# mandt-lab/PSLD

Measured on AMD Instinct MI355X. Metric: train images/sec, CIFAR-10 PSLD (6ch 32x32) NCSN++ HSM step, higher is better.
Workload: dtype f32

## Files before the change

### psld_amd/csrc/conv_wino.hip

```cpp
#include <cstdlib>
#include <cstring>
#include <type_traits>

#include "common.h"
#include "psld_hip.h"
#include "tile_shared.h"
#include "limb.h"

namespace {

constexpr int WT = 32;
constexpr int VPLANE = WT * ROWB;
constexpr int VBYTES = 16 * 3 * VPLANE;
constexpr int WINO_THREADS = 512;

struct WinoArgs {
    const float* x1;
    const float* x2;
    int C1, C2;
    int B, H, W;
    const u32x4* ufrag;
    int N, M;
    int chunks;
    float* C;
    int ldc;
    int nseg, rps;
    int cw;
    PsldEpilogue e;
    const float* zero;
    int nmajor;
    int tiles_m;
    int stagger;
    const float *gsc1, *gsh1, *gsc2, *gsh2;
    int gn_act;
    unsigned long long* dbg;
    int lg_tiles_x, lg_tps;
    int ksplit;
    long long slab_stride;
    int lg_ksplit, lg_xblocks;
    int lg_rpi;
    int mul_seg, mul_w2;
    int rb_img;
    float opscale;
};

constexpr int wino_mul16(int d) { return 65536 / d + 1; }
__host__ __device__ constexpr int wino_div16(int x, int mul) { return (x * mul) >> 16; }
constexpr int WINO_GEOS[6][2] = {{4, 8}, {8, 8}, {16, 8}, {4, 16}, {8, 16}, {4, 32}};
constexpr bool wino_div16_exact() {
    for (const auto& g : WINO_GEOS) {
        const int W2 = g[1] + 2, seg_px = (g[0] + 2) * W2;
        for (int x = 0; x < 256; ++x)
            if (wino_div16(x, wino_mul16(seg_px)) != x / seg_px || wino_div16(x, wino_mul16(W2)) != x / W2) return false;
    }
    return true;
}
static_assert(wino_div16_exact(), "halo decomposition: multiply-shift must equal the division for every pixel below 256");
constexpr bool wino_geo_listed(int rps, int cw) {
    for (const auto& g : WINO_GEOS)
        if (g[0] == rps && g[1] == cw) return true;
    return false;
}
constexpr int wino_lg2(int v) {
    int l = 0;
    while ((1 << l) < v) ++l;
    return (1 << l) == v ? l : -1;
}

__device__ __forceinline__ int raw_off(int hp, int q) {
    return (hp >> 1) * 256 + (((((hp & 1) ^ ((hp >> 1) & 1)) << 3) + q) << 4);
}

template <int NL = 3>
__device__ __forceinline__ void wino_pack_item(const float* __restrict__ w, u32x4* __restrict__ out, long long it, int k_in,
                                               long long sn, long long sk, int flip) {
    const int chunks = k_in / 32;
    long long t = it;
    const int lane = (int)(t & 63); t >>= 6;
    const int chunk = (int)(t % chunks); t /= chunks;
    const int nblk = (int)t;
    const int n = nblk * 16 + (lane & 15);
    const int k0 = chunk * 32 + (lane >> 4) * 8;
    float U[8][16];
#pragma unroll
    for (int j = 0; j < 8; ++j) {
        const float* p = w + n * sn + (k0 + j) * sk;
        float g[3][3];
#pragma unroll
        for (int a = 0; a < 3; ++a)
#pragma unroll
            for (int b = 0; b < 3; ++b) g[a][b] = flip ? p[8 - (a * 3 + b)] : p[a * 3 + b];
        float t4[4][3];
#pragma unroll
        for (int b = 0; b < 3; ++b) {
            t4[0][b] = g[0][b];
            t4[1][b] = 0.5f * ((g[0][b] + g[2][b]) + g[1][b]);
            t4[2][b] = 0.5f * ((g[0][b] + g[2][b]) - g[1][b]);
            t4[3][b] = g[2][b];
        }
#pragma unroll
        for (int a = 0; a < 4; ++a) {
            U[j][a * 4 + 0] = t4[a][0];
            U[j][a * 4 + 1] = 0.5f * ((t4[a][0] + t4[a][2]) + t4[a][1]);
            U[j][a * 4 + 2] = 0.5f * ((t4[a][0] + t4[a][2]) - t4[a][1]);
            U[j][a * 4 + 3] = t4[a][2];
        }
    }
    u32x4* o = out + ((long long)nblk * chunks + chunk) * (16 * NL * 64) + lane;
#pragma unroll
    for (int p = 0; p < 16; ++p) {
        unsigned hi[4], mid[4], lo[4];
#pragma unroll
        for (int j = 0; j < 4; ++j) {
            if constexpr (NL == 3) split3(U[2 * j][p], U[2 * j + 1][p], hi[j], mid[j], lo[j]);
            else if constexpr (NL == 2) split2(U[2 * j][p], U[2 * j + 1][p], hi[j], mid[j]);
            else hi[j] = cvt_pk_f16(U[2 * j][p], U[2 * j + 1][p]);
        }
        o[(p * NL + 0) * 64] = u32x4{hi[0], hi[1], hi[2], hi[3]};
        if constexpr (NL >= 2) o[(p * NL + 1) * 64] = u32x4{mid[0], mid[1], mid[2], mid[3]};
        if constexpr (NL == 3) o[(p * 3 + 2) * 64] = u32x4{lo[0], lo[1], lo[2], lo[3]};
    }
}

template <int NL = 3>
__global__ void wino_pack_kernel(const float* __restrict__ w, u32x4* __restrict__ out, int n_out, int k_in,
                                 long long sn, long long sk, int flip) {
    const long long items = (long long)(n_out / 16) * (k_in / 32) * 64;
    for (long long it = (long long)blockIdx.x * blockDim.x + threadIdx.x; it < items; it += (long long)gridDim.x * blockDim.x)
        wino_pack_item<NL>(w, out, it, k_in, sn, sk, flip);
}

template <int NL = 3>
__global__ void wino_pack_batch_kernel(const long long* __restrict__ tab, int ntab, long long total) {
    for (long long idx = (long long)blockIdx.x * blockDim.x + threadIdx.x; idx < total;
         idx += (long long)gridDim.x * blockDim.x) {
        int lo = 0, hi = ntab - 1;
        while (lo < hi) {
            const int mid = (lo + hi + 1) >> 1;
            if (tab[8 * mid + 7] <= idx) lo = mid; else hi = mid - 1;
        }
        const long long* d = tab + 8 * lo;
        wino_pack_item<NL>(reinterpret_cast<const float*>(d[0]), reinterpret_cast<u32x4*>(d[1]), idx - d[7], (int)d[3], d[5], d[6],
                       (int)d[4]);
    }
}

template <int ABL = 0, bool GNF = false, bool ERAW = false, int LA = 2, bool TAIL = false, int NL = 3, bool SH = false>
__global__ void __launch_bounds__(WINO_THREADS) wino_conv8s_kernel(const WinoArgs a) {
    extern __shared__ __attribute__((aligned(16))) unsigned char smem[];
    constexpr int NI = 4;
    constexpr int RAWB = NI * 64 * 128;
    unsigned char* Vs = smem;
    unsigned char* Rs = smem + VBYTES / 3 * NL;

    const int tid = threadIdx.x;
    const int lane = tid & 63, wave = __builtin_amdgcn_readfirstlane(tid >> 6);
    const int tiles_n = TAIL ? (a.N + 127) >> 7 : a.N >> 7;
    const int nsp = a.ksplit > 1 ? a.ksplit : 1;
    const int tiles_m = a.tiles_m;
    const int per_range = tiles_m * tiles_n;
    const int vb = xcd_remap(blockIdx.x, gridDim.x);
    const int split = nsp > 1 ? vb / per_range : 0;
    const int bid = vb - split * per_range;
    const int kch = a.chunks >> a.lg_ksplit, ch0 = split * kch;
    float* const Cw = a.C + split * a.slab_stride;
    const int tile_n = a.nmajor ? bid / tiles_m : bid % tiles_n;
    const int tile_m = a.nmajor ? bid - tile_n * tiles_m : bid / tiles_n;
    const int n0 = tile_n * 128;
    const bool live = !TAIL || n0 + wave * 16 < a.N;

    const int HW = a.H * a.W;
    const int W2 = a.cw + 2;
    const int lg_tx = a.lg_tiles_x, lg_tps = a.lg_tps;
    const int rpi = HW >= 128 ? HW >> 7 : 1;
    const int tm_img = a.lg_rpi >= 0 ? tile_m >> a.lg_rpi : tile_m / rpi;
    const int reg = tile_m - tm_img * rpi;
    const int img0 = HW >= 128 ? tm_img : tile_m * a.nseg;
    const int oy0 = (reg >> a.lg_xblocks) * a.rps, ox0 = (reg & ((1 << a.lg_xblocks) - 1)) * a.cw;
    const float* zp = a.zero;

    const int c4 = tid & 7;
    int hoff[NI], rdst[NI];
    {
        const int seg_px = (a.rps + 2) * W2;
#pragma unroll
        for (int i = 0; i < NI; ++i) {
            const int px = (tid + WINO_THREADS * i) >> 3;
            const int seg = wino_div16(px, a.mul_seg);
            const int rem = px - seg * seg_px;
            const int hr = wino_div16(rem, a.mul_w2), hx = rem - hr * W2;
            const int img = img0 + seg, iy = oy0 + hr - 1, ix = ox0 + hx - 1;
            const bool ok = seg < a.nseg && img < a.B && iy >= 0 && iy < a.H && ix >= 0 && ix < a.W;
            hoff[i] = ok ? (img * a.H + iy) * a.W + ix : -1;
            rdst[i] = raw_off(px, c4);
        }
    }
    f32x4 hv[NI];
    auto load_raw = [&](int c) {
        const int c0 = c * 32;
        const bool second = c0 >= a.C1;
        const float* src = second ? a.x2 : a.x1;
        const int cs = second ? a.C2 : a.C1;
        const int cc = (second ? c0 - a.C1 : c0) + c4 * 4;
#pragma unroll
        for (int i = 0; i < NI; ++i) hv[i] = ld4(hoff[i] >= 0 ? src + ((long long)hoff[i] * cs + cc) : zp);
    };
    auto store_raw = [&](int buf, int c) {
        if constexpr (GNF) {
            const int c0 = c * 32;
            const bool second = c0 >= a.C1;
            const int cs = second ? a.C2 : a.C1;
            const long long go = (long long)img0 * cs + (second ? c0 - a.C1 : c0) + c4 * 4;
            const f32x4 sc = ld4((second ? a.gsc2 : a.gsc1) + go), sh = ld4((second ? a.gsh2 : a.gsh1) + go);
#pragma unroll
            for (int i = 0; i < NI; ++i) {
                f32x4 o;
#pragma unroll
                for (int e = 0; e < 4; ++e) {
                    const float z = hv[i][e] * sc[e] + sh[e];
                    const float v = a.gn_act ? silu_f(z) : z;
                    o[e] = hoff[i] >= 0 ? v : 0.f;
                }
                *reinterpret_cast<f32x4*>(Rs + buf * RAWB + rdst[i]) = o;
            }
        } else {
#pragma unroll
            for (int i = 0; i < NI; ++i) *reinterpret_cast<f32x4*>(Rs + buf * RAWB + rdst[i]) = hv[i];
        }
    };

    const int vr = wave >> 2;
    const int t_tile = (tid & 255) >> 3, t_q = tid & 7;
    int t_src;
    {
        const int seg = t_tile >> lg_tps, rem = t_tile & ((1 << lg_tps) - 1);
        const int ty = rem >> lg_tx, tx = rem & ((1 << lg_tx) - 1);
        t_src = (seg * (a.rps + 2) + 2 * ty) * W2 + 2 * tx;
    }
    const int t_dst = t_tile * ROWB + (((t_q >> 1) ^ lds_swz(t_tile)) << 4) + (t_q & 1) * 8;
    int t_ro[3][4];
#pragma unroll
    for (int k = 0; k < 3; ++k)
#pragma unroll
        for (int c = 0; c < 4; ++c) {
            t_ro[k][c] = raw_off(t_src + (vr + k) * W2 + c, t_q);
            asm volatile("" : "+v"(t_ro[k][c]));
        }
    auto transform = [&](auto TH, auto VR, int rbuf) {
        constexpr int th = decltype(TH)::value, v_r = decltype(VR)::value;
        constexpr int ra_ = th == 0 ? (v_r == 0 ? 0 : 1) : (v_r == 0 ? 2 : 1);
        constexpr int rb_ = th == 0 ? 2 : (v_r == 0 ? 1 : 3);
        constexpr bool plus = th == 0 && v_r == 1;
        constexpr int vrow = 2 * th + v_r;
        const unsigned char* Rb = Rs + rbuf * RAWB;
        f32x4 ea[4], eb[4];
#pragma unroll
        for (int c = 0; c < 4; ++c) {
            ea[c] = *reinterpret_cast<const f32x4*>(Rb + t_ro[ra_ - v_r][c]);
            eb[c] = *reinterpret_cast<const f32x4*>(Rb + t_ro[rb_ - v_r][c]);
        }
        f32x4 r[4];
#pragma unroll
        for (int c = 0; c < 4; ++c) r[c] = plus ? ea[c] + eb[c] : ea[c] - eb[c];
#pragma unroll
        for (int j = 0; j < 4; ++j) {
            const f32x4 v = j == 0 ? r[0] - r[2] : j == 1 ? r[1] + r[2] : j == 2 ? r[2] - r[1] : r[1] - r[3];
            unsigned h0, m0_, l0, h1, m1, l1;
            if constexpr (NL == 3) {
                split3(v[0], v[1], h0, m0_, l0);
                split3(v[2], v[3], h1, m1, l1);
            } else if constexpr (NL == 2) {
                split2(v[0], v[1], h0, m0_);
                split2(v[2], v[3], h1, m1);
            } else if constexpr (SH) {
                h0 = cvt_pk_f16(v[0] * a.opscale, v[1] * a.opscale);
                h1 = cvt_pk_f16(v[2] * a.opscale, v[3] * a.opscale);
            } else {
                h0 = cvt_pk_f16(v[0], v[1]);
                h1 = cvt_pk_f16(v[2], v[3]);
            }
            unsigned char* q = Vs + (vrow * 4 + j) * NL * VPLANE + t_dst;
            *reinterpret_cast<u32x2*>(q) = u32x2{h0, h1};
            if constexpr (NL >= 2) *reinterpret_cast<u32x2*>(q + VPLANE) = u32x2{m0_, m1};
            if constexpr (NL == 3) *reinterpret_cast<u32x2*>(q + 2 * VPLANE) = u32x2{l0, l1};
        }
    };

    const int r16 = lane & 15, kq = lane >> 4;
    int aoff[2];
#pragma unroll
    for (int tb = 0; tb < 2; ++tb) {
        const int row = tb * 16 + r16;
        aoff[tb] = row * ROWB + ((kq ^ lds_swz(row)) << 4);
    }
    const u32x4* ub = a.ufrag + ((long long)(tile_n * 8 + ((ABL & 128) ? (wave & 3) : wave)) * a.chunks + ch0) * (16 * NL * 64);
    u32x4 bq[4][NL];
    auto load_b = [&](int sigma, u32x4 (&dst)[NL]) {
        const u32x4* p = ub + (long long)sigma * (NL * 64);
#pragma unroll
        for (int l = 0; l < NL; ++l) dst[l] = p[l * 64 + lane];
    };
    f32x4v acc[16][2];
#pragma unroll
    for (int p = 0; p < 16; ++p)
#pragma unroll
        for (int tb = 0; tb < 2; ++tb) acc[p][tb] = f32x4v{0.f, 0.f, 0.f, 0.f};
    u32x4 fa[NL == 1 ? 2 : NL][2];
    auto read_a = [&](int p, int l) {
#pragma unroll
        for (int tb = 0; tb < 2; ++tb) fa[l][tb] = *reinterpret_cast<const u32x4*>(Vs + (p * NL + l) * VPLANE + aoff[tb]);
    };
    auto mm = [&](int p, int la, int lb) {
#pragma unroll
        for (int tb = 0; tb < 2; ++tb) {
            if constexpr (NL == 1)
                acc[p][tb] = __builtin_amdgcn_mfma_f32_16x16x32_f16(
                    __builtin_bit_cast(f16x8, bq[p & 3][lb]), __builtin_bit_cast(f16x8, fa[la][tb]), acc[p][tb], 0, 0, 0);
            else
                acc[p][tb] = __builtin_amdgcn_mfma_f32_16x16x32_bf16(
                    __builtin_bit_cast(bf16x8, bq[p & 3][lb]), __builtin_bit_cast(bf16x8, fa[la][tb]), acc[p][tb], 0, 0, 0);
        }
    };
    auto mfma_half = [&](auto HH, auto LAST, int c) {
        constexpr int h = decltype(HH)::value;
        constexpr bool last = decltype(LAST)::value;
        if constexpr ((ABL & 256) != 0) __builtin_amdgcn_s_setprio(2);
        if constexpr (NL == 1) {
            auto read_a1 = [&](int p) {
#pragma unroll
                for (int tb = 0; tb < 2; ++tb) fa[p & 1][tb] = *reinterpret_cast<const u32x4*>(Vs + p * VPLANE + aoff[tb]);
            };
            read_a1(8 * h);
#pragma unroll
            for (int i = 0; i < 8; ++i) {
                const int p = 8 * h + i;
                if (!(last && p + LA >= 16)) load_b(c * 16 + p + LA, bq[(p + LA) & 3]);
                if (i < 7) read_a1(p + 1);
                __builtin_amdgcn_sched_barrier(0);
                mm(p, p & 1, 0);
                __builtin_amdgcn_sched_barrier(0);
            }
            return;
        }
        if constexpr (NL == 3) read_a(8 * h, 2);
        if constexpr (NL >= 2) read_a(8 * h, 1);
        read_a(8 * h, 0);
#pragma unroll
        for (int i = 0; i < 8; ++i) {
            const int p = 8 * h + i;
            if (!(ABL & 2) && !(last && p + LA >= 16)) load_b(c * 16 + p + LA, bq[(p + LA) & 3]);
            __builtin_amdgcn_sched_barrier(0);
            if constexpr (NL == 3) {
                mm(p, 2, 0);
                __builtin_amdgcn_sched_barrier(0);
                if (i < 7) read_a(p + 1, 2);
                __builtin_amdgcn_sched_barrier(0);
                mm(p, 1, 1);
            }
            if constexpr (NL >= 2) {
                mm(p, 1, 0);
                __builtin_amdgcn_sched_barrier(0);
                if (i < 7) read_a(p + 1, 1);
                __builtin_amdgcn_sched_barrier(0);
            }
            if constexpr (NL == 3) mm(p, 0, 2);
            if constexpr (NL >= 2) mm(p, 0, 1);
            mm(p, 0, 0);
            __builtin_amdgcn_sched_barrier(0);
            if (i < 7) read_a(p + 1, 0);
        }
        if constexpr ((ABL & 256) != 0) __builtin_amdgcn_s_setprio(0);
    };
    using I0 = std::integral_constant<int, 0>;
    using I1 = std::integral_constant<int, 1>;
    if constexpr ((ABL & 4) == 0 && (ABL & 256) == 0) { if (vr != 0) __builtin_amdgcn_s_setprio(1); }

    load_raw(ch0);
    if (live) {
        load_b(0, bq[0]);
        load_b(1, bq[1]);
        if (LA > 2) load_b(2, bq[2]);
    }
    store_raw(0, ch0);
    if constexpr (ERAW) load_raw(ch0 + min(1, kch - 1));
    __syncthreads();
    if (vr == 0) transform(I0{}, I0{}, 0); else transform(I0{}, I1{}, 0);
    __syncthreads();

    auto stamp = [&](int c, int idx) {
        if constexpr ((ABL & 64) != 0) {
            if (c == 3 && a.dbg) {
                __builtin_amdgcn_sched_barrier(0);
                const unsigned long long t = __builtin_amdgcn_s_memtime();
                if (lane == 0) a.dbg[((long long)blockIdx.x * 8 + wave) * 8 + idx] = t;
                __builtin_amdgcn_sched_barrier(0);
            }
        }
    };
    using No = std::false_type;
    using Yes = std::true_type;

    for (int c = 0; c < kch - 1; ++c) {
        stamp(c, 0);
        if constexpr (!ERAW) load_raw(ch0 + c + 1);
        if (vr == 0 && !(ABL & 1)) transform(I1{}, I0{}, c & 1);
        __builtin_amdgcn_sched_barrier(0);
        if (vr == 0) stamp(c, 1);
        if (live) mfma_half(I0{}, No{}, c);
        __builtin_amdgcn_sched_barrier(0);
        if (vr != 0) stamp(c, 1);
        if (vr != 0 && !(ABL & 1)) transform(I1{}, I1{}, c & 1);
        stamp(c, 2);
        store_raw((c + 1) & 1, ch0 + c + 1);
        stamp(c, 3);
        __syncthreads();
        stamp(c, 4);
        if (vr == 0 && !(ABL & 1)) transform(I0{}, I0{}, (c + 1) & 1);
        __builtin_amdgcn_sched_barrier(0);
        if (vr == 0) stamp(c, 5);
        if (live) mfma_half(I1{}, No{}, c);
        __builtin_amdgcn_sched_barrier(0);
        if (vr != 0) stamp(c, 5);
        if constexpr (ERAW) load_raw(ch0 + min(c + 2, kch - 1));
        if (vr != 0 && !(ABL & 1)) transform(I0{}, I1{}, (c + 1) & 1);
        stamp(c, 6);
        __syncthreads();
        stamp(c, 7);
    }
    {
        int c = kch - 1;
        asm volatile("" : "+s"(c));
        stamp(c, 0);
        if (vr == 0 && !(ABL & 1)) transform(I1{}, I0{}, c & 1);
        __builtin_amdgcn_sched_barrier(0);
        if (vr == 0) stamp(c, 1);
        if (live) mfma_half(I0{}, No{}, c);
        __builtin_amdgcn_sched_barrier(0);
        if (vr != 0) stamp(c, 1);
        if (vr != 0 && !(ABL & 1)) transform(I1{}, I1{}, c & 1);
        stamp(c, 2);
        stamp(c, 3);
        __syncthreads();
        stamp(c, 4);
        __builtin_amdgcn_sched_barrier(0);
        stamp(c, 5);
        if (live) mfma_half(I1{}, Yes{}, c);
// ... 483 lines not shown
```

### psld_amd/csrc/pointwise.hip

```cpp
#include "common.h"
#include "psld_hip.h"

namespace {

inline int grid_for(long long n, int per_thread = 1) {
    long long b = (n + 256LL * per_thread - 1) / (256LL * per_thread);
    if (b > 256LL * 16) b = 256LL * 16;
    if (b < 1) b = 1;
    return (int)b;
}

#define GRID_STRIDE(i, n) \
    for (long long i = (long long)blockIdx.x * blockDim.x + threadIdx.x; i < (n); i += (long long)gridDim.x * blockDim.x)

__global__ void transpose_kernel(const float* __restrict__ x, float* __restrict__ y, int rows, int cols) {
    __shared__ float tile[32][33];
    const long long img = blockIdx.z;
    const float* xp = x + img * rows * cols;
    float* yp = y + img * rows * cols;
    const int c0 = blockIdx.x * 32, r0 = blockIdx.y * 32;
    const int tx = threadIdx.x & 31, ty = threadIdx.x >> 5;
    for (int j = ty; j < 32; j += 8) {
        const int r = r0 + j, c = c0 + tx;
        if (r < rows && c < cols) tile[j][tx] = xp[(long long)r * cols + c];
// ... 207 lines not shown
        const float* p = job.src + col;
        const long long step = 16ll * job.ld;
        int r = lane;
        for (; r + 7 * 16 < job.rows; r += 8 * 16) {
            float v[8];
            const float* q = p + (long long)r * job.ld;
#pragma unroll
            for (int u = 0; u < 8; ++u) v[u] = q[u * step];
#pragma unroll
            for (int u = 0; u < 8; ++u) acc += (double)v[u];
        }
        for (; r < job.rows; r += 16) acc += (double)p[(long long)r * job.ld];
    }
    sh[lane * 64 + (tid & 63)] = acc;
    __syncthreads();
    if (lane == 0 && col < job.c) {
        double t = 0.0;
#pragma unroll
        for (int l = 0; l < 16; ++l) t += sh[l * 64 + tid];
        const float v = (float)(t * (double)job.alpha);
        job.dst1[col] = v;
        if (job.dst2) job.dst2[col] = v;
    }
}

__global__ void im2col3x3_small_kernel(const float* __restrict__ x, int ih, int iw, int c, int oh, int ow, int stride,
                                       int pad, int flip, float* __restrict__ out, int ld_out, long long total) {
    GRID_STRIDE(i, total) {
        const int j = (int)(i % ld_out);
        const long long m = i / ld_out;
        float v = 0.f;
        if (j < 9 * c) {
            const int ch = j / 9;
            int t = j - ch * 9;
            if (flip) t = 8 - t;
            const int ky = t / 3, kx = t - ky * 3;
            const int ox = (int)(m % ow);
            const long long r = m / ow;
            const int oy = (int)(r % oh);
            const long long n = r / oh;
            const int iy = oy * stride + ky - pad, ix = ox * stride + kx - pad;
            if (iy >= 0 && iy < ih && ix >= 0 && ix < iw) v = x[((n * ih + iy) * iw + ix) * c + ch];
        }
        out[i] = v;
    }
}

__global__ void im2col3x3_kernel(const float* __restrict__ x, int ih, int iw, int c4, int oh, int ow, int stride, int pad,
                                 float* __restrict__ cols, long long total4) {
    GRID_STRIDE(i, total4) {
        const int q = (int)(i % c4);
        long long r = i / c4;
        const int t = (int)(r % 9);
        const long long m = r / 9;
        const int ky = t / 3, kx = t - ky * 3;
        const int ox = (int)(m % ow);
        const long long rr = m / ow;
        const int oy = (int)(rr % oh);
        const long long n = rr / oh;
        const int iy = oy * stride + ky - pad, ix = ox * stride + kx - pad;
        f32x4 v = {0.f, 0.f, 0.f, 0.f};
        if (iy >= 0 && iy < ih && ix >= 0 && ix < iw)
            v = reinterpret_cast<const f32x4*>(x)[((n * ih + iy) * iw + ix) * c4 + q];
        reinterpret_cast<f32x4*>(cols)[i] = v;
    }
}
__global__ void col2im3x3_kernel(const float* __restrict__ dcols, int ih, int iw, int c4, int oh, int ow, int stride,
                                 int pad, float* __restrict__ dx, long long total4) {
    GRID_STRIDE(i, total4) {
        const int q = (int)(i % c4);
        long long r = i / c4;
        const int ix = (int)(r % iw);
        r /= iw;
        const int iy = (int)(r % ih);
        const long long n = r / ih;
        f32x4 acc = {0.f, 0.f, 0.f, 0.f};
#pragma unroll
        for (int ky = 0; ky < 3; ++ky) {
            const int ty = iy + pad - ky;
            if (ty < 0 || ty % stride) continue;
            const int oy = ty / stride;
            if (oy >= oh) continue;
#pragma unroll
            for (int kx = 0; kx < 3; ++kx) {
                const int tx = ix + pad - kx;
                if (tx < 0 || tx % stride) continue;
                const int ox = tx / stride;
                if (ox >= ow) continue;
                const long long m = (n * oh + oy) * ow + ox;
                acc += reinterpret_cast<const f32x4*>(dcols)[(m * 9 + ky * 3 + kx) * c4 + q];
            }
        }
        reinterpret_cast<f32x4*>(dx)[i] = acc;
    }
}

template <int COUT>
__global__ void __launch_bounds__(256) conv3x3_fewout_kernel(const float* __restrict__ x, const float* __restrict__ w_ohwi,
                                                            const float* __restrict__ bias, float* __restrict__ y,
                                                            int batch, int h, int w, int c) {
    extern __shared__ __attribute__((aligned(16))) float wl[];
    for (int i = threadIdx.x; i < 9 * COUT * c; i += blockDim.x) {
        const int ch = i % c, r = i / c;
        const int o = r % COUT, t = r / COUT;
        wl[i] = w_ohwi[((long long)o * 9 + t) * c + ch];
    }
    __syncthreads();
    const int lane = threadIdx.x & 63, wave = threadIdx.x >> 6;
    const int c4 = c >> 2;
    const bool live = lane < c4;
    const int wq = (w + 3) >> 2;
    const long long groups = (long long)batch * h * wq;
    for (long long gidx = (long long)blockIdx.x * 4 + wave; gidx < groups; gidx += (long long)gridDim.x * 4) {
        const int gx = (int)(gidx % wq);
        const long long r = gidx / wq;
        const int oy = (int)(r % h);
        const long long n = r / h;
        const int ox0 = gx * 4;
        f32x4 win[3][6];
#pragma unroll
        for (int dy = 0; dy < 3; ++dy)
#pragma unroll
            for (int dx = 0; dx < 6; ++dx) {
                const int iy = oy + dy - 1, ix = ox0 + dx - 1;
                const bool ok = live && iy >= 0 && iy < h && ix >= 0 && ix < w;
                win[dy][dx] = ok ? reinterpret_cast<const f32x4*>(x)[((n * h + iy) * w + ix) * c4 + lane]
                                 : f32x4{0.f, 0.f, 0.f, 0.f};
            }
        float acc[4][COUT];
#pragma unroll
        for (int p = 0; p < 4; ++p)
#pragma unroll
            for (int o = 0; o < COUT; ++o) acc[p][o] = 0.f;
        if (live) {
#pragma unroll
            for (int t = 0; t < 9; ++t) {
                const int ky = t / 3, kx = t - ky * 3;
#pragma unroll
                for (int o = 0; o < COUT; ++o) {
                    const f32x4 wv = *reinterpret_cast<const f32x4*>(wl + ((t * COUT + o) * c) + lane * 4);
#pragma unroll
                    for (int p = 0; p < 4; ++p) {
                        const f32x4 xv = win[ky][p + kx];
                        float a = acc[p][o];
                        a = fmaf(xv[0], wv[0], a);
                        a = fmaf(xv[1], wv[1], a);
                        a = fmaf(xv[2], wv[2], a);
                        a = fmaf(xv[3], wv[3], a);
                        acc[p][o] = a;
                    }
                }
            }
        }
#pragma unroll
        for (int p = 0; p < 4; ++p)
#pragma unroll
            for (int o = 0; o < COUT; ++o) {
                float v = acc[p][o];
#pragma unroll
                for (int sft = 32; sft >= 1; sft >>= 1) v += __shfl_xor(v, sft, 64);
                acc[p][o] = v;
            }
        if (lane < 4 && ox0 + lane < w) {
            float* yo = y + (((n * h + oy) * w + ox0 + lane) * COUT);
#pragma unroll
            for (int o = 0; o < COUT; ++o) {
                float v = lane == 0 ? acc[0][o] : lane == 1 ? acc[1][o] : lane == 2 ? acc[2][o] : acc[3][o];
                yo[o] = v + (bias ? bias[o] : 0.f);
            }
        }
    }
}

__global__ void copy_batch_kernel(const long long* __restrict__ tab, int ntab, long long total4) {
    GRID_STRIDE(i, total4) {
        int lo = 0, hi = ntab - 1;
        while (lo < hi) {
            const int mid = (lo + hi + 1) >> 1;
            if (tab[4 * mid + 3] <= i) lo = mid; else hi = mid - 1;
        }
        const long long* d = tab + 4 * lo;
        const long long j = i - d[3];
        reinterpret_cast<f32x4*>(d[1])[j] = reinterpret_cast<const f32x4*>(d[0])[j];
    }
}

__global__ void scale_copy2d_kernel(const float* __restrict__ src, int ld_src, float* __restrict__ dst, int ld_dst,
                                    long long rows, int cols, float alpha) {
    GRID_STRIDE(i, rows * cols) {
        const long long r = i / cols;
        const int j = (int)(i - r * cols);
        dst[r * ld_dst + j] = alpha * src[r * ld_src + j];
    }
}

__global__ void axpby_kernel(const float* __restrict__ a, float sa, const float* __restrict__ b, float sb,
                             float* __restrict__ y, long long n4, long long n, int accumulate) {
    GRID_STRIDE(i, n4) {
        f32x4 v = reinterpret_cast<const f32x4*>(a)[i] * sa;
        if (b) v += reinterpret_cast<const f32x4*>(b)[i] * sb;
        if (accumulate) v += reinterpret_cast<const f32x4*>(y)[i];
        reinterpret_cast<f32x4*>(y)[i] = v;
    }
    const long long t0 = n4 * 4;
    GRID_STRIDE(j, n - t0) {
        const long long i = t0 + j;
        float v = a[i] * sa;
        if (b) v += b[i] * sb;
        if (accumulate) v += y[i];
        y[i] = v;
    }
}

__global__ void copy2d_kernel(const float* __restrict__ src, int ld_src, float* __restrict__ dst, int ld_dst,
                              long long rows, int cols4, int accumulate) {
    const long long n = rows * cols4;
    GRID_STRIDE(i, n) {
        const long long r = i / cols4;
        const int c = (int)(i - r * cols4) * 4;
        f32x4 v = *reinterpret_cast<const f32x4*>(src + r * ld_src + c);
        float* d = dst + r * ld_dst + c;
        if (accumulate) v += *reinterpret_cast<const f32x4*>(d);
        *reinterpret_cast<f32x4*>(d) = v;
    }
}

__global__ void silu_kernel(const float* __restrict__ x, float* __restrict__ y, long long n) {
    GRID_STRIDE(i, n) y[i] = silu_f(x[i]);
}
__global__ void silu_bwd_kernel(const float* __restrict__ x, const float* __restrict__ dy, float* __restrict__ dx,
                                long long n) {
    GRID_STRIDE(i, n) dx[i] = dy[i] * dsilu_f(x[i]);
}

__global__ void colsum_partial_kernel(const float* __restrict__ x, int ld, int hw, int c, int cq, int pl,
                                      int chunk_px, int chunks, double* __restrict__ part) {
    extern __shared__ double red[];
    const int b = blockIdx.y, chunk = blockIdx.x;
    const int q = threadIdx.x % cq, l = threadIdx.x / cq;
    const int p0 = chunk * chunk_px, p1 = min(hw, p0 + chunk_px);
    const float* base = x + ((long long)b * hw) * ld + q * 4;
    f32x4 acc = {0.f, 0.f, 0.f, 0.f};
#pragma unroll 4
    for (int p = p0 + l; p < p1; p += pl) acc += *reinterpret_cast<const f32x4*>(base + (long long)p * ld);
#pragma unroll
    for (int e = 0; e < 4; ++e) red[(long long)l * cq * 4 + q * 4 + e] = (double)acc[e];
    __syncthreads();
    for (int i = threadIdx.x; i < cq * 4; i += blockDim.x) {
        double t = 0.0;
        for (int ll = 0; ll < pl; ++ll) t += red[(long long)ll * cq * 4 + i];
        part[((long long)b * chunks + chunk) * c + i] = t;
    }
}
__global__ void colsum_final_kernel(const double* __restrict__ part, int chunks, int c, float* __restrict__ out,
                                    float alpha, int ld_out) {
    const int b = blockIdx.y;
    const int col = blockIdx.x * blockDim.x + threadIdx.x;
    if (col >= c) return;
    double t = 0.0;
    for (int k = 0; k < chunks; ++k) t += part[((long long)b * chunks + k) * c + col];
    out[(long long)b * ld_out + col] = (float)(t * (double)alpha);
}
__global__ void __launch_bounds__(1024) colsum_final_total_kernel(const double* __restrict__ part, int chunks, int batch,
                                                                  int c, float* __restrict__ per_image, int ld,
                                                                  float* __restrict__ out, float alpha,
                                                                  float* __restrict__ out1 = nullptr,
                                                                  float* __restrict__ out2 = nullptr, int seg = 0) {
    __shared__ double red[64][16];
    const int cl = threadIdx.x & 15, bl = threadIdx.x >> 4;
    const int col = blockIdx.x * 16 + cl;
    double tot = 0.0;
    if (col < c)
        for (int b = bl; b < batch; b += 64) {
            const double* p = part + (long long)b * chunks * c + col;
            double t = 0.0;
#pragma unroll 8
            for (int k = 0; k < chunks; ++k) t += p[(long long)k * c];
            const float f = (float)t;
            per_image[(long long)b * ld + col] = f;
            tot += (double)f;
        }
    red[bl][cl] = tot;
    __syncthreads();
    if (bl == 0 && col < c) {
        double t = 0.0;
#pragma unroll
        for (int l = 0; l < 64; ++l) t += red[l][cl];
        const float v = (float)(t * (double)alpha);
        if (seg <= 0 || col < seg) out[col] = v;
        else if (col < 2 * seg) out1[col - seg] = v;
        else out2[col - 2 * seg] = v;
    }
}
__global__ void colsum_kernel(const float* __restrict__ x, int ld, int hw, int c, float* __restrict__ out,
                              float alpha) {
    __shared__ double red[4][64];
    const int b = blockIdx.y;
    const int col = blockIdx.x * 64 + (threadIdx.x & 63);
    const int rl = threadIdx.x >> 6;
    double acc = 0.0;
    if (col < c) {
        const float* p = x + ((long long)b * hw) * ld + col;
        float part = 0.f;
        int cnt = 0;
        for (int r = rl; r < hw; r += 4) {
            part += p[(long long)r * ld];
            if (++cnt == 32) {
                acc += (double)part;
                part = 0.f;
                cnt = 0;
            }
        }
        acc += (double)part;
    }
    red[rl][threadIdx.x & 63] = acc;
    __syncthreads();
    if (rl == 0 && col < c) out[(long long)b * c + col] = (float)((red[0][threadIdx.x] + red[1][threadIdx.x] + red[2][threadIdx.x] + red[3][threadIdx.x]) * (double)alpha);
}

template <int V>
__global__ void softmax_rows_reg_kernel(const float* __restrict__ x, float* __restrict__ y, long long rows, int L) {
    const long long row = (long long)blockIdx.x * (blockDim.x >> 6) + (threadIdx.x >> 6);
    if (row >= rows) return;
    const int lane = threadIdx.x & 63;
    const f32x4* xp = reinterpret_cast<const f32x4*>(x + row * L);
    f32x4 v[V];
    float mx = -INFINITY;
#pragma unroll
    for (int j = 0; j < V; ++j) {
        v[j] = xp[lane + 64 * j];
        mx = fmaxf(mx, fmaxf(fmaxf(v[j][0], v[j][1]), fmaxf(v[j][2], v[j][3])));
    }
    mx = wave_max(mx);
    float s = 0.f;
#pragma unroll
    for (int j = 0; j < V; ++j)
#pragma unroll
        for (int e = 0; e < 4; ++e) {
            v[j][e] = expf(v[j][e] - mx);
            s += v[j][e];
        }
    s = wave_sum(s);
    const float inv = 1.0f / s;
    f32x4* yp = reinterpret_cast<f32x4*>(y + row * L);
#pragma unroll
    for (int j = 0; j < V; ++j) yp[lane + 64 * j] = v[j] * inv;
}
template <int V>
__global__ void softmax_rows_bwd_reg_kernel(const float* __restrict__ y, const float* __restrict__ dy,
                                            float* __restrict__ dx, long long rows, int L) {
    const long long row = (long long)blockIdx.x * (blockDim.x >> 6) + (threadIdx.x >> 6);
    if (row >= rows) return;
    const int lane = threadIdx.x & 63;
    const f32x4* yp = reinterpret_cast<const f32x4*>(y + row * L);
    const f32x4* gp = reinterpret_cast<const f32x4*>(dy + row * L);
    f32x4 yv[V], gv[V];
    double d = 0.0;
#pragma unroll
    for (int j = 0; j < V; ++j) {
        yv[j] = yp[lane + 64 * j];
        gv[j] = gp[lane + 64 * j];
#pragma unroll
        for (int e = 0; e < 4; ++e) d = fma((double)yv[j][e], (double)gv[j][e], d);
    }
    d = wave_sum_d(d);
    f32x4* op = reinterpret_cast<f32x4*>(dx + row * L);
#pragma unroll
    for (int j = 0; j < V; ++j) {
        f32x4 o;
#pragma unroll
        for (int e = 0; e < 4; ++e) o[e] = yv[j][e] * (float)((double)gv[j][e] - d);
        op[lane + 64 * j] = o;
    }
}

__global__ void softmax_rows_kernel(const float* __restrict__ x, float* __restrict__ y, long long rows, int L) {
    const long long row = (long long)blockIdx.x * (blockDim.x >> 6) + (threadIdx.x >> 6);
    if (row >= rows) return;
    const int lane = threadIdx.x & 63;
    const float* xp = x + row * L;
    float* yp = y + row * L;
    float mx = -INFINITY;
    for (int i = lane; i < L; i += 64) mx = fmaxf(mx, xp[i]);
    mx = wave_max(mx);
    float s = 0.f;
    for (int i = lane; i < L; i += 64) {
        const float e = expf(xp[i] - mx);
        yp[i] = e;
        s += e;
    }
    s = wave_sum(s);
    const float inv = 1.0f / s;
    for (int i = lane; i < L; i += 64) yp[i] *= inv;
}

__global__ void softmax_rows_bwd_kernel(const float* __restrict__ y, const float* __restrict__ dy,
                                        float* __restrict__ dx, long long rows, int L) {
    const long long row = (long long)blockIdx.x * (blockDim.x >> 6) + (threadIdx.x >> 6);
    if (row >= rows) return;
    const int lane = threadIdx.x & 63;
    const float* yp = y + row * L;
    const float* gp = dy + row * L;
    double d = 0.0;
    for (int i = lane; i < L; i += 64) d = fma((double)yp[i], (double)gp[i], d);
    d = wave_sum_d(d);
    for (int i = lane; i < L; i += 64) dx[row * L + i] = yp[i] * (float)((double)gp[i] - d);
}

__global__ void time_embed_kernel(const float* __restrict__ t, const float* __restrict__ W, float* __restrict__ out,
                                  int batch, int e, int use_log) {
    const int i = blockIdx.x * blockDim.x + threadIdx.x;
    if (i >= batch * e) return;
    const int b = i / e, k = i % e;
    float p;
    if (use_log) {
        const float lt = logf(t[b]);
        p = __fmul_rn(__fmul_rn(__fmul_rn(lt, W[k]), 2.0f), 3.14159265358979323846f);
    } else {
        p = __fmul_rn(t[b], W[k]);
    }
    out[(long long)b * 2 * e + k] = sinf(p);
    out[(long long)b * 2 * e + e + k] = cosf(p);
}

__global__ void samples_to_u8_kernel(const double* __restrict__ x, unsigned char* __restrict__ out, int batch,
                                     int c, int c_total, int hw, int denorm) {
    const long long n = (long long)batch * hw * c;
    GRID_STRIDE(i, n) {
        const int ch = (int)(i % c);
        long long t = i / c;
        const int p = (int)(t % hw);
        const int b = (int)(t / hw);
        double v = x[((long long)b * c_total + ch) * hw + p];
        if (denorm) v = v * 0.5 + 0.5;
        v = v * 255.0;
        v = v < 0.0 ? 0.0 : (v > 255.0 ? 255.0 : v);
        out[i] = (unsigned char)v;
    }
}
__global__ void u8_to_images_kernel(const unsigned char* __restrict__ img, float* __restrict__ out,
                                    const unsigned char* __restrict__ flip, int batch, int c, int h, int w, int norm) {
    const long long n = (long long)batch * c * h * w;
    GRID_STRIDE(i, n) {
        const int xw = (int)(i % w);
        long long t = i / w;
        const int y = (int)(t % h);
        t /= h;
        const int ch = (int)(t % c);
        const int b = (int)(t / c);
        const int sx = (flip && flip[b]) ? (w - 1 - xw) : xw;
        const double u = (double)img[(((long long)b * h + y) * w + sx) * c + ch];
        out[i] = (float)(norm ? (u / 127.5) - 1.0 : u / 255.0);
    }
}

__global__ void f64_to_f32_kernel(const double* __restrict__ x, float* __restrict__ y, long long n) {
    GRID_STRIDE(i, n) y[i] = (float)x[i];
}
__global__ void f32_to_f64_kernel(const float* __restrict__ x, double* __restrict__ y, long long n) {
    GRID_STRIDE(i, n) y[i] = (double)x[i];
}

}

extern "C" int psld_nchw_to_nhwc_f32(const float* x, float* y, int batch, int c, int hw, hipStream_t stream) {
    PSLD_CHECK_ARG(x && y && batch > 0 && c > 0 && hw > 0, "psld_nchw_to_nhwc_f32: bad args");
    hipLaunchKernelGGL(transpose_kernel, dim3(cdiv(hw, 32), cdiv(c, 32), batch), dim3(256), 0, stream, x, y, c, hw);
    PSLD_CHECK_LAUNCH("psld_nchw_to_nhwc_f32");
    return PSLD_OK;
}
extern "C" int psld_nhwc_to_nchw_f32(const float* x, float* y, int batch, int c, int hw, hipStream_t stream) {
    PSLD_CHECK_ARG(x && y && batch > 0 && c > 0 && hw > 0, "psld_nhwc_to_nchw_f32: bad args");
    hipLaunchKernelGGL(transpose_kernel, dim3(cdiv(c, 32), cdiv(hw, 32), batch), dim3(256), 0, stream, x, y, hw, c);
    PSLD_CHECK_LAUNCH("psld_nhwc_to_nchw_f32");
    return PSLD_OK;
}

extern "C" int psld_pack_oihw_to_ohwi_f32(const float* w, float* out, int cout, int cin, int taps, hipStream_t stream) {
    PSLD_CHECK_ARG(w && out, "psld_pack_oihw_to_ohwi_f32: null pointer");
    const long long n = (long long)cout * cin * taps;
    hipLaunchKernelGGL(pack_ohwi_kernel, dim3(grid_for(n)), dim3(256), 0, stream, w, out, cout, cin, taps);
    PSLD_CHECK_LAUNCH("psld_pack_oihw_to_ohwi_f32");
    return PSLD_OK;
}
extern "C" int psld_pack_oihw_to_dgrad_f32(const float* w, float* out, int cout, int cin, int taps, hipStream_t stream) {
    PSLD_CHECK_ARG(w && out, "psld_pack_oihw_to_dgrad_f32: null pointer");
    const long long n = (long long)cout * cin * taps;
    hipLaunchKernelGGL(pack_dgrad_kernel, dim3(grid_for(n)), dim3(256), 0, stream, w, out, cout, cin, taps);
    PSLD_CHECK_LAUNCH("psld_pack_oihw_to_dgrad_f32");
    return PSLD_OK;
}
extern "C" int psld_reduce_slabs_f32(const float* slabs, int nsplit, long long n, float* out, int layout, int cout,
                                     int taps, int cin, float alpha, hipStream_t stream) {
    PSLD_CHECK_ARG(slabs && out && nsplit >= 1, "psld_reduce_slabs_f32: bad args");
    PSLD_CHECK_ARG(layout == 0 || n == (long long)cout * taps * cin, "psld_reduce_slabs_f32: shape mismatch");
    const bool vec = n % 4 == 0 && (layout == 0 || cin % 4 == 0) && (reinterpret_cast<uintptr_t>(slabs) & 15) == 0 &&
                     (layout == 1 || (reinterpret_cast<uintptr_t>(out) & 15) == 0);
    if (vec)
        hipLaunchKernelGGL(reduce_slabs4_kernel, dim3(grid_for(n / 4)), dim3(256), 0, stream, slabs, nsplit, n, out, layout,
                           taps, cin, alpha);
    else
        hipLaunchKernelGGL(reduce_slabs_kernel, dim3(grid_for(n)), dim3(256), 0, stream, slabs, nsplit, n, out, layout,
                           taps, cin, alpha);
    PSLD_CHECK_LAUNCH("psld_reduce_slabs_f32");
    return PSLD_OK;
}

extern "C" int psld_reduce_slabs_batch_units(long long n, int layout, int taps, int cin) {
    if (n <= 0 || n % 4) return 0;
    if (layout == 1) {
        if (taps < 1 || taps > RSB_MAXTAPS || cin < 4 || cin % 4 || n % ((long long)taps * cin)) return 0;
        return (int)(n / ((long long)taps * cin)) * ((cin + RSB_CI - 1) / RSB_CI);
    }
    if (layout == 2 && (taps < 4 || taps % 4 || cin < taps || cin % 4 || n % taps)) return 0;
    return (int)((n / 4 + RSB_FLAT4 - 1) / RSB_FLAT4);
}

extern "C" int psld_reduce_slabs_batch_f32(const long long* table_dev, int jobs, long long units, hipStream_t stream) {
    PSLD_CHECK_ARG(table_dev && jobs > 0 && units > 0 && units < (1ll << 31), "psld_reduce_slabs_batch_f32: bad args");
    hipLaunchKernelGGL(reduce_slabs_batch_kernel, dim3((unsigned)units), dim3(256), 0, stream, table_dev, jobs);
    PSLD_CHECK_LAUNCH("psld_reduce_slabs_batch_f32");
    return PSLD_OK;
}

extern "C" int psld_param_reduce2_f32(const float* src_a, const float* src_b, int rows, int ld, int c, float* dst_a,
                                      float* dst_b, float alpha, hipStream_t stream) {
    PSLD_CHECK_ARG(src_a && dst_a && rows > 0 && c > 0 && ld >= c && (!src_b) == (!dst_b), "psld_param_reduce2_f32: bad args");
    const ParamJob ja{src_a, rows, ld, c, dst_a, nullptr, alpha}, jb{src_b, rows, ld, c, dst_b, nullptr, alpha};
    const int per = cdiv(c, 64);
    hipLaunchKernelGGL(param_reduce_kernel, dim3(src_b ? 2 * per : per), dim3(1024), 0, stream, nullptr, 0, ja, jb, per);
    PSLD_CHECK_LAUNCH("psld_param_reduce2_f32");
    return PSLD_OK;
}

extern "C" int psld_param_reduce_batch_f32(const long long* table_dev, int jobs, int blocks, hipStream_t stream) {
    PSLD_CHECK_ARG(table_dev && jobs > 0 && blocks > 0, "psld_param_reduce_batch_f32: bad args");
    const ParamJob none{nullptr, 0, 0, 0, nullptr, nullptr, 0.f};
    hipLaunchKernelGGL(param_reduce_kernel, dim3(blocks), dim3(1024), 0, stream, table_dev, jobs, none, none, 0);
    PSLD_CHECK_LAUNCH("psld_param_reduce_batch_f32");
    return PSLD_OK;
}

extern "C" int psld_im2col3x3_small_f32(const float* x, int batch, int ih, int iw, int c, int oh, int ow, int stride,
                                        int pad, int flip, float* out, int ld_out, hipStream_t stream) {
    PSLD_CHECK_ARG(x && out && batch > 0 && c > 0 && 9 * c <= ld_out && oh > 0 && ow > 0 && stride >= 1,
                   "psld_im2col3x3_small_f32: bad args (c=%d ld_out=%d)", c, ld_out);
    PSLD_CHECK_ARG(!flip || stride == 1, "psld_im2col3x3_small_f32: flip needs stride 1");
    const long long total = (long long)batch * oh * ow * ld_out;
    hipLaunchKernelGGL(im2col3x3_small_kernel, dim3(grid_for(total)), dim3(256), 0, stream, x, ih, iw, c, oh, ow, stride,
                       pad, flip, out, ld_out, total);
    PSLD_CHECK_LAUNCH("psld_im2col3x3_small_f32");
    return PSLD_OK;
}

extern "C" int psld_im2col3x3_f32(const float* x, int batch, int ih, int iw, int c, int oh, int ow, int stride, int pad,
                                  float* cols, hipStream_t stream) {
    PSLD_CHECK_ARG(x && cols && batch > 0 && c > 0 && c % 4 == 0 && oh > 0 && ow > 0 && stride >= 1 && pad >= 0 &&
                       (reinterpret_cast<uintptr_t>(x) & 15) == 0 && (reinterpret_cast<uintptr_t>(cols) & 15) == 0,
                   "psld_im2col3x3_f32: bad args (c=%d)", c);
    const long long total4 = (long long)batch * oh * ow * 9 * (c / 4);
    hipLaunchKernelGGL(im2col3x3_kernel, dim3(grid_for(total4)), dim3(256), 0, stream, x, ih, iw, c / 4, oh, ow, stride, pad,
                       cols, total4);
    PSLD_CHECK_LAUNCH("psld_im2col3x3_f32");
    return PSLD_OK;
}

extern "C" int psld_col2im3x3_f32(const float* dcols, int batch, int ih, int iw, int c, int oh, int ow, int stride, int pad,
                                  float* dx, hipStream_t stream) {
    PSLD_CHECK_ARG(dcols && dx && batch > 0 && c > 0 && c % 4 == 0 && oh > 0 && ow > 0 && stride >= 1 && pad >= 0 &&
                       (reinterpret_cast<uintptr_t>(dx) & 15) == 0 && (reinterpret_cast<uintptr_t>(dcols) & 15) == 0,
                   "psld_col2im3x3_f32: bad args (c=%d)", c);
    const long long total4 = (long long)batch * ih * iw * (c / 4);
    hipLaunchKernelGGL(col2im3x3_kernel, dim3(grid_for(total4)), dim3(256), 0, stream, dcols, ih, iw, c / 4, oh, ow, stride,
                       pad, dx, total4);
    PSLD_CHECK_LAUNCH("psld_col2im3x3_f32");
    return PSLD_OK;
}

extern "C" int psld_conv3x3_fewout_supported(int cin, int cout) {
    return cin > 0 && cin % 4 == 0 && cin <= 256 && (cout == 3 || cout == 6) && 9 * cout * cin * 4 <= 64 * 1024;
}

extern "C" int psld_conv3x3_fewout_f32(const float* x, const float* w_ohwi, const float* bias, float* y, int batch,
                                       int h, int w, int cin, int cout, hipStream_t stream) {
    PSLD_CHECK_ARG(x && w_ohwi && y && batch > 0 && h > 0 && w > 0, "psld_conv3x3_fewout_f32: bad args");
    PSLD_CHECK_ARG(psld_conv3x3_fewout_supported(cin, cout), "psld_conv3x3_fewout_f32: unsupported cin=%d cout=%d", cin, cout);
    PSLD_CHECK_ARG((reinterpret_cast<uintptr_t>(x) & 15) == 0, "psld_conv3x3_fewout_f32: unaligned input");
    const size_t lds = (size_t)9 * cout * cin * sizeof(float);
    const long long groups = (long long)batch * h * ((w + 3) / 4);
    long long blocks = (groups + 3) / 4;
    if (blocks > 2048) blocks = 2048;
    if (cout == 6) {
        static PsldPerDeviceFlag configured_; bool& configured = configured_.here();
        if (!configured) {
            (void)hipFuncSetAttribute(reinterpret_cast<const void*>(&conv3x3_fewout_kernel<6>),
                                      hipFuncAttributeMaxDynamicSharedMemorySize, 64 * 1024);
            configured = true;
        }
        hipLaunchKernelGGL(conv3x3_fewout_kernel<6>, dim3((unsigned)blocks), dim3(256), lds, stream, x, w_ohwi, bias, y, batch,
                           h, w, cin);
    } else {
        static PsldPerDeviceFlag configured_; bool& configured = configured_.here();
        if (!configured) {
            (void)hipFuncSetAttribute(reinterpret_cast<const void*>(&conv3x3_fewout_kernel<3>),
                                      hipFuncAttributeMaxDynamicSharedMemorySize, 64 * 1024);
            configured = true;
        }
        hipLaunchKernelGGL(conv3x3_fewout_kernel<3>, dim3((unsigned)blocks), dim3(256), lds, stream, x, w_ohwi, bias, y, batch,
                           h, w, cin);
    }
    PSLD_CHECK_LAUNCH("psld_conv3x3_fewout_f32");
    return PSLD_OK;
}

extern "C" int psld_copy_batch_f32(const long long* table_dev, int entries, long long total4, hipStream_t stream) {
// ... 250 lines not shown
```

Before: 1255.

## Stage Winograd weight packing through shared memory and unroll colsum loads

The batched Winograd weight-pack kernel now processes one 64-lane unit per wave. It loads the 16x32x9 weight block with coalesced 16-byte loads into a padded LDS tile, then each lane reads its 8x9 filters from LDS. This replaces strided per-thread global gathers, and the generic per-item path is kept as a fallback for misaligned or odd-stride cases. Separately, colsum batches 8 independent loads before accumulating to expose memory-level parallelism, keeping the same 32-element float partials flushed to double.

```diff
diff --git a/psld_amd/csrc/conv_wino.hip b/psld_amd/csrc/conv_wino.hip
--- a/psld_amd/csrc/conv_wino.hip
+++ b/psld_amd/csrc/conv_wino.hip
@@ -122,6 +122,84 @@
     }
 }
 
+constexpr int WPK_RS_N = 292;
+constexpr int WPK_RS_K = 148;
+constexpr int WPK_TILE = 32 * WPK_RS_K > 16 * WPK_RS_N ? 32 * WPK_RS_K : 16 * WPK_RS_N;
+template <int NL, bool ROWS_N>
+__device__ __forceinline__ void wino_pack_unit(const float* __restrict__ w, u32x4* __restrict__ out, int unit, int k_in,
+                                               long long sn, long long sk, int flip, float* tile) {
+    constexpr int RS = ROWS_N ? WPK_RS_N : WPK_RS_K;
+    const int lane = threadIdx.x & 63;
+    const int chunks = k_in / 32;
+    const int chunk = unit % chunks, nblk = unit / chunks;
+    const unsigned char* src = reinterpret_cast<const unsigned char*>(w + (long long)nblk * 16 * sn + (long long)chunk * 32 * sk);
+    const unsigned rsb = (unsigned)(ROWS_N ? sn : sk) * 4;
+    constexpr int HEAD4 = ROWS_N ? 64 : 32, REST4 = ROWS_N ? 8 : 4;
+    const unsigned hrow = ROWS_N ? 0u : (unsigned)(lane >> 5), hcol = ROWS_N ? (unsigned)lane : (unsigned)(lane & 31);
+    f32x4 v[18];
+#pragma unroll
+    for (int i = 0; i < 16; ++i) {
+        const unsigned r0 = ROWS_N ? i : 2 * i;
+        v[i] = *reinterpret_cast<const f32x4*>(src + ((r0 + hrow) * rsb + hcol * 16));
+    }
+#pragma unroll
+    for (int t = 0; t < 2; ++t) {
+        const unsigned e = (unsigned)lane + 64 * t, r = e / REST4, c4 = HEAD4 + e % REST4;
+        v[16 + t] = *reinterpret_cast<const f32x4*>(src + (r * rsb + c4 * 16));
+    }
+#pragma unroll
+    for (int i = 0; i < 16; ++i) {
+        const unsigned r0 = ROWS_N ? i : 2 * i;
+        *reinterpret_cast<f32x4*>(tile + (r0 + hrow) * RS + hcol * 4) = v[i];
+    }
+#pragma unroll
+    for (int t = 0; t < 2; ++t) {
+        const unsigned e = (unsigned)lane + 64 * t, r = e / REST4, c4 = HEAD4 + e % REST4;
+        *reinterpret_cast<f32x4*>(tile + r * RS + c4 * 4) = v[16 + t];
+    }
+    __syncthreads();
+    const float* mine = tile + (lane & 15) * (ROWS_N ? RS : 9) + (lane >> 4) * 8 * (ROWS_N ? 9 : RS);
+    float g[8][9];
+#pragma unroll
+    for (int j = 0; j < 8; ++j)
+#pragma unroll
+        for (int t = 0; t < 9; ++t) g[j][t] = mine[j * (ROWS_N ? 9 : RS) + (flip ? 8 - t : t)];
+    __syncthreads();
+    u32x4* o = out + (long long)unit * (16 * NL * 64) + lane;
+#pragma unroll
+    for (int a = 0; a < 4; ++a) {
+        float U[8][4];
+#pragma unroll
+        for (int j = 0; j < 8; ++j) {
+            float t4[3];
+#pragma unroll
+            for (int b = 0; b < 3; ++b)
+                t4[b] = a == 0   ? g[j][b]
+                        : a == 1 ? 0.5f * ((g[j][b] + g[j][6 + b]) + g[j][3 + b])
+                        : a == 2 ? 0.5f * ((g[j][b] + g[j][6 + b]) - g[j][3 + b])
+                                 : g[j][6 + b];
+            U[j][0] = t4[0];
+            U[j][1] = 0.5f * ((t4[0] + t4[2]) + t4[1]);
+            U[j][2] = 0.5f * ((t4[0] + t4[2]) - t4[1]);
+            U[j][3] = t4[2];
+        }
+#pragma unroll
+        for (int pp = 0; pp < 4; ++pp) {
+            const int p = a * 4 + pp;
+            unsigned hi[4], mid[4], lo[4];
+#pragma unroll
+            for (int j = 0; j < 4; ++j) {
+                if constexpr (NL == 3) split3(U[2 * j][pp], U[2 * j + 1][pp], hi[j], mid[j], lo[j]);
+                else if constexpr (NL == 2) split2(U[2 * j][pp], U[2 * j + 1][pp], hi[j], mid[j]);
+                else hi[j] = cvt_pk_f16(U[2 * j][pp], U[2 * j + 1][pp]);
+            }
+            o[(p * NL + 0) * 64] = u32x4{hi[0], hi[1], hi[2], hi[3]};
+            if constexpr (NL >= 2) o[(p * NL + 1) * 64] = u32x4{mid[0], mid[1], mid[2], mid[3]};
+            if constexpr (NL == 3) o[(p * 3 + 2) * 64] = u32x4{lo[0], lo[1], lo[2], lo[3]};
+        }
+    }
+}
+
 template <int NL = 3>
 __global__ void wino_pack_kernel(const float* __restrict__ w, u32x4* __restrict__ out, int n_out, int k_in,
                                  long long sn, long long sk, int flip) {
@@ -131,17 +209,43 @@
 }
 
 template <int NL = 3>
-__global__ void wino_pack_batch_kernel(const long long* __restrict__ tab, int ntab, long long total) {
-    for (long long idx = (long long)blockIdx.x * blockDim.x + threadIdx.x; idx < total;
-         idx += (long long)gridDim.x * blockDim.x) {
-        int lo = 0, hi = ntab - 1;
-        while (lo < hi) {
-            const int mid = (lo + hi + 1) >> 1;
-            if (tab[8 * mid + 7] <= idx) lo = mid; else hi = mid - 1;
-        }
-        const long long* d = tab + 8 * lo;
-        wino_pack_item<NL>(reinterpret_cast<const float*>(d[0]), reinterpret_cast<u32x4*>(d[1]), idx - d[7], (int)d[3], d[5], d[6],
-                       (int)d[4]);
+__global__ void __launch_bounds__(64, 2) wino_pack_batch_kernel(const long long* __restrict__ tab, int ntab, long long total) {
+    __shared__ __attribute__((aligned(16))) float tile[WPK_TILE];
+    long long first = 0, next = 0;
+    const long long* d = tab;
+    for (long long base = (long long)blockIdx.x * 64; base < total; base += (long long)gridDim.x * 64) {
+        if (base >= next) {
+            int lo = 0, hi = ntab - 1;
+            while (lo < hi) {
+                const int mid = (lo + hi + 1) >> 1;
+                if (tab[8 * mid + 7] <= base) lo = mid; else hi = mid - 1;
+            }
+            d = tab + 8 * lo;
+            first = d[7];
+            next = lo + 1 < ntab ? tab[8 * (lo + 1) + 7] : total;
+        }
+        const float* w = reinterpret_cast<const float*>(d[0]);
+        u32x4* out = reinterpret_cast<u32x4*>(d[1]);
+        const int k_in = (int)d[3], flip = (int)d[4];
+        const long long sn = d[5], sk = d[6];
+        const bool whole = base + 64 <= next && ((base - first) & 63) == 0 && (reinterpret_cast<uintptr_t>(w) & 15) == 0;
+        if (whole && sk == 9 && (sn & 3) == 0) {
+            wino_pack_unit<NL, true>(w, out, (int)((base - first) >> 6), k_in, sn, sk, flip, tile);
+        } else if (whole && sn == 9 && (sk & 3) == 0) {
+            wino_pack_unit<NL, false>(w, out, (int)((base - first) >> 6), k_in, sn, sk, flip, tile);
+        } else {
+            const long long idx = base + threadIdx.x;
+            if (idx < total) {
+                int lo = 0, hi = ntab - 1;
+                while (lo < hi) {
+                    const int mid = (lo + hi + 1) >> 1;
+                    if (tab[8 * mid + 7] <= idx) lo = mid; else hi = mid - 1;
+                }
+                const long long* di = tab + 8 * lo;
+                wino_pack_item<NL>(reinterpret_cast<const float*>(di[0]), reinterpret_cast<u32x4*>(di[1]), idx - di[7], (int)di[3],
+                                   di[5], di[6], (int)di[4]);
+            }
+        }
     }
 }
 
diff --git a/psld_amd/csrc/pointwise.hip b/psld_amd/csrc/pointwise.hip
--- a/psld_amd/csrc/pointwise.hip
+++ b/psld_amd/csrc/pointwise.hip
@@ -533,15 +533,20 @@
     if (col < c) {
         const float* p = x + ((long long)b * hw) * ld + col;
         float part = 0.f;
-        int cnt = 0;
-        for (int r = rl; r < hw; r += 4) {
-            part += p[(long long)r * ld];
-            if (++cnt == 32) {
-                acc += (double)part;
-                part = 0.f;
-                cnt = 0;
+        int r = rl;
+        for (; r + 4 * 31 < hw; r += 128) {
+#pragma unroll
+            for (int g8 = 0; g8 < 4; ++g8) {
+                float v[8];
+#pragma unroll
+                for (int k = 0; k < 8; ++k) v[k] = p[(long long)(r + 4 * (8 * g8 + k)) * ld];
+#pragma unroll
+                for (int k = 0; k < 8; ++k) part += v[k];
             }
-        }
+            acc += (double)part;
+            part = 0.f;
+        }
+        for (; r < hw; r += 4) part += p[(long long)r * ld];
         acc += (double)part;
     }
     red[rl][threadIdx.x & 63] = acc;
```

After: 1260 (median of 6 runs). No clear change (+0.4%).
